# apache/arrow-go

Hardware: AMD Instinct MI355X
Metric: GB/s processed per kernel (Sum/Add/Filter/Take) vs HBM roofline (higher is better)
Workload: dtype int64+f64

## Files before the change

### arrow_go_amd/csrc/ah_common.h

```cpp
#pragma once
#include <hip/hip_runtime.h>
#include <initializer_list>
#include <type_traits>
#include <stdarg.h>
#include <stdint.h>
#include <stddef.h>
#include <stdio.h>
#include <stdlib.h>
#include <string.h>
#include "../../include/arrowhip.h"

#define AH_EXPORT extern "C" __attribute__((visibility("default")))

struct ah_filter_cache {
  bool valid;
  const uint8_t *fdata, *fvalid;
  int64_t foff, n, ntiles;
  int null_sel, tile_rows;
  void* buf;
  size_t bytes;
  int64_t* super_off;
  int* tile_local;
  int64_t* total;
};
// ... 71 lines not shown
static inline int ah_fail(ah_ctx* ctx, int code, const char* fmt, ...) {
  if (ctx) {
    va_list ap;
    va_start(ap, fmt);
    vsnprintf(ctx->err, sizeof(ctx->err), fmt, ap);
    va_end(ap);
  }
  return code;
}

#define AH_HIP(ctx, call)                                                              \
  do {                                                                                 \
    hipError_t e__ = (call);                                                           \
    if (e__ != hipSuccess)                                                             \
      return ah_fail((ctx), AH_EHIP, "%s failed: %s (%s:%d)", #call, hipGetErrorString(e__), \
                     __FILE__, __LINE__);                                              \
  } while (0)

#define AH_ENTER_KEEP(ctx)                                             \
  do {                                                                 \
    if (!(ctx)) return AH_EINVALID;                                    \
    (ctx)->err[0] = 0;                                                 \
    AH_HIP((ctx), hipSetDevice((ctx)->device));                        \
  } while (0)

#define AH_ENTER(ctx)                                                  \
  do {                                                                 \
    AH_ENTER_KEEP(ctx);                                                \
    (ctx)->fcache.valid = false;                                       \
    (ctx)->take_hint_valid = false;                                    \
  } while (0)

static inline bool ah_take_hint_overlaps(const ah_ctx* c, const void* p, size_t nbytes) {
  if (!c->take_hint_valid || !c->take_hint_idx) return false;
  const uintptr_t a = (uintptr_t)p, b = a + nbytes, lo = (uintptr_t)c->take_hint_idx, hi = lo + (size_t)c->take_hint_nidx * (size_t)(c->take_hint_kind / 2);
  return a < hi && lo < b;
}
static inline bool ah_fcache_overlaps(const ah_ctx* c, const void* p, size_t nbytes) {
  if (!c->fcache.valid) return false;
  const uintptr_t a = (uintptr_t)p, b = a + nbytes;
  const uintptr_t lo = (uintptr_t)(c->fcache.foff >> 3), hi = (uintptr_t)((c->fcache.foff + c->fcache.n + 7) >> 3);
  for (const uint8_t* bm : {c->fcache.fdata, c->fcache.fvalid})
    if (bm && a < (uintptr_t)bm + hi && (uintptr_t)bm + lo < b) return true;
  return false;
}

#define AH_LAUNCH_CHECK(ctx) AH_HIP((ctx), hipGetLastError())

void ah_expr_cache_free(ah_ctx* ctx);
int ah_arith_binary(ah_ctx* ctx, int type, int op, int shape, const void* l, const void* r, void* out, int64_t len);
int ah_partition_by_group(ah_ctx* ctx, const int32_t* ids, const unsigned long long* vals, const uint8_t* vvalid, int64_t voff, int64_t n,
                          int shift, int passes, unsigned* hist, unsigned* offs, unsigned long long* alt_vals, unsigned* alt_ids,
                          unsigned long long* out_vals, unsigned* out_ids);
int ah_sort_rest_msd(ah_ctx* ctx, unsigned long long* keys, unsigned* rows, unsigned long long* alt_keys, unsigned* alt_rows, int64_t n,
                     unsigned long long varying, unsigned long long kmin, unsigned long long kmax, int float_bytes, int descending, void* tmp,
                     unsigned long long* out64, int* used);
size_t ah_sort_msd_temp_bytes(int64_t n);
int ah_sort_pairs_lsd(ah_ctx* ctx, unsigned long long* keys, unsigned* rows, unsigned long long* alt_keys, unsigned* alt_rows, int64_t n,
                      unsigned* hist, unsigned* offs, unsigned long long** sorted_keys);
int ah_take_binned_try(ah_ctx* ctx, int byte_width, const void* values, const uint8_t* vvalid, int64_t voff, int64_t nvalues, int iw,
                       int is_signed, const void* idx, const uint8_t* ivalid, int64_t ioff, int64_t nidx, void* out_values,
                       uint8_t* out_valid, unsigned long long* first_bad, int* used);
int ah_groupby_partitioned_try(ah_ctx* ctx, int is_f64, const uint64_t* keys, const uint8_t* kvalid, int64_t koff, const void* vals,
                               const uint8_t* vvalid, int64_t voff, int64_t n, uint64_t* out_keys, void* out_sums, int64_t* out_counts,
                               int64_t* out_first_rows, int64_t* out_ngroups, int32_t* out_null_group, int* used);
int ah_fused_f64_parts_dev(ah_ctx* ctx, int cmpop, const double* x, const uint8_t* valid, int64_t off, int64_t n, double threshold,
                           double* out_sum_dev, int64_t* out_count_dev, double* out_parts_dev);
size_t ah_sum_partial_bytes(int is_f64);
int ah_sum_chunk_partials(ah_ctx* ctx, int is_f64, const void* buf, size_t len, void* partials, int max_partials, int* n_written);
int ah_sum_finish_partials(ah_ctx* ctx, int is_f64, const void* partials, int n, void* res_dev);
int ah_sum_short_f64(ah_ctx* ctx, const void* buf, size_t len, void* res_dev);
int ah_encode_partitioned_try(ah_ctx* ctx, const uint64_t* keys, const uint8_t* valid, int64_t off, int64_t n, int encode_nulls, int lp, int slots,
                              int32_t* out_ids, uint64_t* out_dict, int64_t* out_first_rows, int64_t* out_ndict, int32_t* out_null_id, int* used);
int ah_encode_u64_groups(ah_ctx* ctx, const uint64_t* keys, const uint8_t* kvalid, int64_t koff, int64_t n, int32_t* ids, uint64_t* out_keys,
                         int64_t* out_first_rows, int64_t* out_ngroups, int32_t* out_null_group);
int ah_encode_u64_first_seen(ah_ctx* ctx, const uint64_t* keys, const uint8_t* valid, int64_t off, int64_t n, int32_t* ids, int64_t* out_first_rows,
                             int64_t* out_ngroups);
int ah_encode_tuple_first_seen(ah_ctx* ctx, int ncols, const ah_group_key* keys, int64_t n, int32_t* ids, int64_t* out_first_rows, int64_t* out_ngroups);
int ah_encode_first_look(ah_ctx* ctx, const uint64_t* keys, const uint8_t* valid, int64_t off, int64_t rows, uint64_t* distinct);
int ah_encode_partitioned2_try(ah_ctx* ctx, const uint64_t* keys, const uint8_t* valid, int64_t off, int64_t n, int encode_nulls, int lp, int slots,
                               int32_t* out_ids, uint64_t* out_dict, int64_t* out_first_rows, int64_t* out_ndict, int32_t* out_null_id, int* used);
int ah_compact_u64_by_bits(ah_ctx* ctx, const uint64_t* values, const uint8_t* bits, int64_t n, uint64_t* out_values, int64_t* out_rows);
int ah_check_stall(ah_ctx* ctx);
int ah_mailbox_read(ah_ctx* ctx, const unsigned long long* dev_words, int nwords, unsigned long long* out_host);
int ah_mailbox_begin(ah_ctx* ctx, unsigned long long** mb_out, unsigned long long* seq_out);
int ah_mailbox_wait(ah_ctx* ctx, unsigned long long seq, int nwords, unsigned long long* out_host);
#if defined(__HIPCC__)
__device__ __forceinline__ void ah_mailbox_post(unsigned long long* mb, unsigned long long seq, const unsigned long long* words, int nwords) {
  for (int i = 0; i < nwords; i++) __hip_atomic_store(&mb[i], words[i], __ATOMIC_RELAXED, __HIP_MEMORY_SCOPE_SYSTEM);
  __hip_atomic_store(&mb[7], seq, __ATOMIC_RELEASE, __HIP_MEMORY_SCOPE_SYSTEM);
}
#endif
int ah_mailbox_read2(ah_ctx* ctx, const unsigned long long* dev_words, int nwords, const unsigned long long* dev_words2, int nwords2,
                     unsigned long long* out_host);
int ah_scratch_reserve(ah_ctx* ctx, size_t nbytes, void** out);
int ah_temp_reserve(ah_ctx* ctx, size_t nbytes, void** out, bool* out_of_memory = nullptr);
int ah_pack_reserve(ah_ctx* ctx, size_t nbytes, void** out);
static inline constexpr size_t ah_pad(size_t b) { return (b + 255) & ~(size_t)255; }
struct TempCarver {
  uint8_t* base = nullptr;
  size_t used = 0;
  uint8_t* take(size_t b) { uint8_t* q = base ? base + used : nullptr; used += ah_pad(b); return q; }
  template <typename T> size_t take(T*& p, size_t count) { p = (T*)take(count * sizeof(T)); return ah_pad(count * sizeof(T)); }
};
constexpr int kDsScalars = 64;
constexpr int kDsSum = 0;
constexpr int kDsFusedSum = 8, kDsFusedCount = 9;
constexpr int kDsMinMax = 12;
constexpr int kDsGbDone = 20;
// ... 210 lines not shown
```

### arrow_go_amd/csrc/ah_sort.hip

```cpp
#include <algorithm>
#include <type_traits>
#include <vector>
#include "ah_sort_radix.h"

namespace {

enum { kCatRest = 0, kCatNaN = 1, kCatNull = 2 };

template <typename T>
__device__ __forceinline__ unsigned long long make_key(T v, bool descending) {
  using U = typename std::make_unsigned<typename std::conditional<std::is_floating_point<T>::value,
                                                                    typename std::conditional<sizeof(T) == 4, int, long long>::type, T>::type>::type;
  constexpr U sign = (U)1 << (sizeof(T) * 8 - 1);
  U k;
  if constexpr (std::is_floating_point<T>::value) {
    if (v == (T)0) v = (T)0;
    U b = __builtin_bit_cast(U, v);
    k = (b & sign) ? (U)~b : (U)(b | sign);
  } else if constexpr (std::is_signed<T>::value) {
    k = (U)v ^ sign;
  } else {
    k = (U)v;
  }
  if (descending) k = (U)~k;
  return (unsigned long long)k;
}

template <typename T>
struct Column {
  const T* values;
  const uint8_t* valid;
  int64_t off;
  int descending, nulls_at_start;
  const unsigned* rows_in;
  __device__ __forceinline__ void load(int64_t i, unsigned long long* key, unsigned* row, unsigned* digit) const {
    const unsigned r = rows_in ? rows_in[i] : (unsigned)i;
    const T v = values[r];
    int cat = kCatRest;
    if (!ah_bit(valid, off + r)) cat = kCatNull;
    else if (std::is_floating_point<T>::value && v != v) cat = kCatNaN;
    *key = cat == kCatRest ? make_key<T>(v, descending) : 0ull;
    *row = r;
    *digit = nulls_at_start ? (unsigned)(2 - cat) : (unsigned)cat;
  }
};
struct IdVal {
  const int32_t* ids;
  const unsigned long long* vals;
  const uint8_t* vvalid;
  int64_t voff;
  int shift;
  __device__ __forceinline__ void load(int64_t i, unsigned long long* key, unsigned* row, unsigned* digit) const {
    const unsigned g = (unsigned)ids[i];
    const bool ok = ah_bit(vvalid, voff + i);
    *key = ok ? vals[i] : 0ull;
    *row = ok ? g : (g | 0x80000000u);
    *digit = (g >> shift) & 255u;
  }
};

struct ValId {
  const unsigned long long* vals;
  const unsigned* ids;
  int shift;
  __device__ __forceinline__ void load(int64_t i, unsigned long long* key, unsigned* row, unsigned* digit) const {
    *key = vals[i];
    *row = ids[i];
    *digit = ((*row & 0x7fffffffu) >> shift) & 255u;
  }
};

template <typename T>
__global__ __launch_bounds__(kBlock) void pairs_kernel(const T* __restrict__ values, int64_t n, int descending, unsigned long long* __restrict__ keys,
                                                        unsigned* __restrict__ rows, unsigned long long* __restrict__ res) {
  KeyStats st;
  st.init();
  constexpr int U = 4;
  const int64_t stride = (int64_t)gridDim.x * kBlock * U;
  for (int64_t base = (int64_t)blockIdx.x * kBlock * U + threadIdx.x; base < n; base += stride) {
    T v[U];
#pragma unroll
    for (int u = 0; u < U; u++) { const int64_t i = base + (int64_t)u * kBlock; v[u] = i < n ? __builtin_nontemporal_load(&values[i]) : (T)0; }
#pragma unroll
    for (int u = 0; u < U; u++) {
      const int64_t i = base + (int64_t)u * kBlock;
      if (i >= n) continue;
      if (std::is_floating_point<T>::value && v[u] != v[u]) { st.nans++; continue; }
      const unsigned long long k = make_key<T>(v[u], descending);
      __builtin_nontemporal_store(k, &keys[i]);
      __builtin_nontemporal_store((unsigned)i, &rows[i]);
      st.add(k);
    }
  }
  st = ah_block_reduce<kBlock>(st);
  if (threadIdx.x == 0) st.store<5>(res + (size_t)blockIdx.x * 5);
}

__global__ __launch_bounds__(kBlock) void emit_kernel(const unsigned* __restrict__ rows, int64_t n, uint64_t* __restrict__ out) {
  const int64_t stride = (int64_t)gridDim.x * kBlock;
  for (int64_t i = (int64_t)blockIdx.x * kBlock + threadIdx.x; i < n; i += stride) out[i] = rows[i];
}


template <typename T>
int sort_by_column(ah_ctx* c, SortBuffers& b, const void* values, const uint8_t* valid, int64_t off, int64_t n, int descending,
                   int nulls_at_start, const unsigned* rows_in) {
  const int64_t ntiles = ah_ceil_div(n, (int64_t)kTile * tiles_per_block(n));
  int rc;
  Column<T> col{(const T*)values, valid, off, descending, nulls_at_start, rows_in};
  int64_t rest_lo = 0, rest_n = 0;
  unsigned long long k_and = ~0ull, k_or = 0, kmin = ~0ull, kmax = 0;
  bool have_stats = false;
  if (valid == nullptr && rows_in == nullptr && n >= ((int64_t)1 << 20)) {
    const unsigned pgrid = std::min(ah_stream_grid(c, ah_ceil_div(n, (int64_t)kBlock * 4), 8), (unsigned)kAndOrGrid);
    pairs_kernel<T><<<pgrid, kBlock, 0, c->stream>>>((const T*)values, n, descending, b.ka, b.ra, b.andor);
    AH_LAUNCH_CHECK(c);
    std::vector<unsigned long long> parts((size_t)pgrid * 5);
    AH_HIP(c, hipMemcpyAsync(parts.data(), b.andor, parts.size() * 8, hipMemcpyDeviceToHost, c->stream));
    AH_HIP(c, hipStreamSynchronize(c->stream));
    unsigned long long nans = 0;
    for (unsigned g = 0; g < pgrid; g++) {
      k_and &= parts[g * 5]; k_or |= parts[g * 5 + 1];
      kmin = parts[g * 5 + 2] < kmin ? parts[g * 5 + 2] : kmin;
      kmax = parts[g * 5 + 3] > kmax ? parts[g * 5 + 3] : kmax;
      nans += parts[g * 5 + 4];
    }
    if (nans == 0) { have_stats = true; rest_lo = 0; rest_n = n; }
  }
  if (!have_stats) {
    if ((rc = radix_pass(c, col, n, b.hist, b.offs, b.ka, b.ra)) != AH_OK) return rc;
    unsigned ends[3];
    for (int d = 0; d < 3; d++)
      AH_HIP(c, hipMemcpyAsync(&c->pinned[d], b.offs + ((int64_t)d + 1) * ntiles - 1, 4, hipMemcpyDeviceToHost, c->stream));
    AH_HIP(c, hipStreamSynchronize(c->stream));
    for (int d = 0; d < 3; d++) ends[d] = *(volatile unsigned*)&c->pinned[d];
    rest_lo = nulls_at_start ? ends[1] : 0;
    rest_n = nulls_at_start ? (int64_t)ends[2] - ends[1] : ends[0];
  }
  unsigned long long *kcur = b.ka + rest_lo, *kalt = b.kb + rest_lo;
  unsigned *rcur = b.ra + rest_lo, *ralt = b.rb + rest_lo;
  if (rest_n > 1) {
    if (!have_stats) {
      const unsigned agrid = std::min(ah_stream_grid(c, ah_ceil_div(rest_n, kBlock), 4), (unsigned)kAndOrGrid);
      and_or_kernel<<<agrid, kBlock, 0, c->stream>>>(kcur, rest_n, b.andor);
      AH_LAUNCH_CHECK(c);
      std::vector<unsigned long long> parts((size_t)agrid * 4);
      AH_HIP(c, hipMemcpyAsync(parts.data(), b.andor, parts.size() * 8, hipMemcpyDeviceToHost, c->stream));
      AH_HIP(c, hipStreamSynchronize(c->stream));
      for (unsigned g = 0; g < agrid; g++) {
        k_and &= parts[g * 4]; k_or |= parts[g * 4 + 1];
        kmin = parts[g * 4 + 2] < kmin ? parts[g * 4 + 2] : kmin;
        kmax = parts[g * 4 + 3] > kmax ? parts[g * 4 + 3] : kmax;
      }
    }
    const unsigned long long varying = k_and ^ k_or;
    int nvar = 0;
    for (int by = 0; by < (int)sizeof(T); by++) nvar += ((varying >> (8 * by)) & 0xFFull) != 0;
    bool done = false;
    if (rows_in == nullptr && nvar >= 4 && c->opt_sort_msd) {
      int used = -1;
      if ((rc = ah_sort_rest_msd(c, kcur, rcur, kalt, ralt, rest_n, varying, kmin, kmax, std::is_floating_point<T>::value ? (int)sizeof(T) : 0, descending, b.msd_tmp,
                                 (unsigned long long*)(rest_n == n ? b.final_out : nullptr), &used)) != AH_OK) return rc;
      if (used > 0) {
        done = true;
        b.emitted = rest_n == n && b.final_out != nullptr;
      } else if (used == 0 && b.msd_tmp && ah_sort_msd_temp_bytes(rest_n) != 0) {
        if ((rc = radix_pass(c, col, n, b.hist, b.offs, b.ka, b.ra)) != AH_OK) return rc;
      }
    }
    for (int by = 0; !done && by < (int)sizeof(T); by++) {
      if (((varying >> (8 * by)) & 0xFFull) == 0) continue;
      Pairs src{kcur, rcur, 8 * by};
      if ((rc = radix_pass(c, src, rest_n, b.hist, b.offs, kalt, ralt)) != AH_OK) return rc;
      unsigned long long* tk = kcur; kcur = kalt; kalt = tk;
      unsigned* tr = rcur; rcur = ralt; ralt = tr;
    }
    if (!b.emitted && rcur != b.ra + rest_lo) AH_HIP(c, hipMemcpyAsync(b.ra + rest_lo, rcur, (size_t)rest_n * 4, hipMemcpyDeviceToDevice, c->stream));
  }
  return AH_OK;
}

int sort_dispatch(ah_ctx* c, SortBuffers& b, const SortCol& k, int64_t n, const unsigned* rows_in) {
  switch (k.type) {
#define AH_SORT(ID, T) case ID: return sort_by_column<T>(c, b, k.values, k.valid, k.off, n, k.descending, k.nulls_at_start, rows_in);
    AH_SORT(AH_UINT8, uint8_t) AH_SORT(AH_INT8, int8_t) AH_SORT(AH_UINT16, uint16_t) AH_SORT(AH_INT16, int16_t)
    AH_SORT(AH_UINT32, uint32_t) AH_SORT(AH_INT32, int32_t) AH_SORT(AH_UINT64, uint64_t) AH_SORT(AH_INT64, int64_t)
    AH_SORT(AH_FLOAT32, float) AH_SORT(AH_FLOAT64, double)
#undef AH_SORT
  }
  if (ah_sort_is_binary(k.type)) return ah_sort_by_binary(c, b, k, n, rows_in);
  return ah_fail(c, AH_ENOTIMPL, "sorting not supported for type %d", k.type);
}

int sort_keys(ah_ctx* c, int nkeys, const SortCol* keys, int64_t n, uint64_t* out) {
  SortBuffers b;
  const int64_t ntiles = ah_ceil_div(n, kTile);
  int rc;
  bool any_binary = false;
  for (int k = 0; k < nkeys; k++) any_binary |= ah_sort_is_binary(keys[k].type);
  const size_t hist_bytes = (size_t)kRadix * ntiles * 4;
  const size_t msd_bytes = c->opt_sort_msd ? ah_sort_msd_temp_bytes(n) : 0;
  const size_t bin_bytes = any_binary ? kBinArrays * Carver::pad((size_t)n * 4) : 0;
  const size_t total = 2 * Carver::pad((size_t)n * 8) + (nkeys > 1 ? 3 : 2) * Carver::pad((size_t)n * 4) + 2 * Carver::pad(hist_bytes) + Carver::pad(4096 * 8 * 8) + Carver::pad(msd_bytes) + bin_bytes;
  void* arena;
  if ((rc = ah_temp_reserve(c, total, &arena)) != AH_OK) return rc;
  Carver tmp{(uint8_t*)arena};
  tmp.take((size_t)n * 8, &b.ka);
  tmp.take((size_t)n * 8, &b.kb);
  tmp.take((size_t)n * 4, &b.ra);
  tmp.take((size_t)n * 4, &b.rb);
  b.rc = nullptr;
  if (nkeys > 1) tmp.take((size_t)n * 4, &b.rc);
  tmp.take(hist_bytes, &b.hist);
  tmp.take(hist_bytes, &b.offs);
  tmp.take((size_t)kAndOrGrid * 8 * 8, &b.andor);
  if (msd_bytes) { uint8_t* m; tmp.take(msd_bytes, &m); b.msd_tmp = m; }
  if (any_binary)
    for (int i = 0; i < kBinArrays; i++) tmp.take((size_t)n * 4, &b.bin[i]);
  const unsigned* rows_in = nullptr;
  if (nkeys == 1) b.final_out = out;
  for (int k = nkeys - 1; k >= 0; k--) {
    if ((rc = sort_dispatch(c, b, keys[k], n, rows_in)) != AH_OK) return rc;
    if (k > 0) {
      AH_HIP(c, hipMemcpyAsync(b.rc, b.ra, (size_t)n * 4, hipMemcpyDeviceToDevice, c->stream));
      rows_in = b.rc;
    }
  }
  if (!b.emitted) {
    emit_kernel<<<ah_stream_grid(c, ah_ceil_div(n, kBlock), 8), kBlock, 0, c->stream>>>(b.ra, n, out);
    AH_LAUNCH_CHECK(c);
  }
  return AH_OK;
}

}

int ah_partition_by_group(ah_ctx* c, const int32_t* ids, const unsigned long long* vals, const uint8_t* vvalid, int64_t voff, int64_t n, int shift,
// ... 99 lines not shown
```

### arrow_go_amd/csrc/ah_sort_msd.hip

```cpp
#include "ah_common.h"
#include "ah_bins.h"
#include "ah_msd.h"

namespace {

constexpr int kLocalMax = 512;
constexpr int kBigMax = 8192, kBigList = 1024;

struct MsMap {
  unsigned long long mask;
  int lshift;
  int fkind, descending;
};
__device__ __forceinline__ double ms_value(unsigned long long u, const MsMap& m) {
  if (m.fkind == 8) {
    const unsigned long long k = m.descending ? ~u : u;
    return __builtin_bit_cast(double, (k >> 63) ? (k & 0x7fffffffffffffffull) : ~k);
  }
  const unsigned k = m.descending ? ~(unsigned)(u >> 32) : (unsigned)(u >> 32);
  return (double)__builtin_bit_cast(float, (k >> 31) ? (k & 0x7fffffffu) : ~k);
}
__device__ __forceinline__ double ms_frac(unsigned long long u, unsigned long long pa, unsigned long long pb, const MsMap& m) {
  if (pb <= pa) return 0.0;
  if (m.fkind && m.lshift == (m.fkind == 8 ? 0 : 32) && ((pa ^ pb) >> 63)) {
    const double xa = ms_value(pa, m), xb = ms_value(pb, m);
    if (xb != xa && xa - xa == 0.0 && xb - xb == 0.0) return (ms_value(u, m) - xa) / (xb - xa);
  }
  return (double)(u - pa) / (double)(pb - pa);
}
constexpr int kSplit = 4096;
constexpr int64_t kSample = (int64_t)1 << 18;

__global__ __launch_bounds__(256) void ms_sample_kernel(const unsigned long long* __restrict__ keys, int64_t n, int64_t stride, int64_t count, MsMap m,
                                                         unsigned long long* __restrict__ sample, unsigned* __restrict__ sample_rows) {
  const int64_t j = (int64_t)blockIdx.x * 256 + threadIdx.x;
  if (j >= count) return;
  const int64_t i = j * stride;
  sample[j] = i < n ? (keys[i] & m.mask) << m.lshift : ~0ull;
  sample_rows[j] = (unsigned)j;
}
struct MsPoints {
  const unsigned long long* sorted;
  int64_t count;
  unsigned long long umin, umax;
  __device__ __forceinline__ unsigned long long at(int64_t i) const { return i <= 0 ? umin : (i > count ? umax : sorted[i - 1]); }
  __device__ __forceinline__ int64_t first(int k) const { return k == 0 ? 0 : 64 * (int64_t)k + 1; }
  __device__ __forceinline__ int64_t last(int k) const { return k == kSplit - 1 ? count + 1 : 64 * (int64_t)(k + 1) + 1; }
};
constexpr int kFlagWords = kSplit / 32;
__global__ __launch_bounds__(256) void ms_split_kernel(MsPoints p, unsigned long long* __restrict__ split, unsigned* __restrict__ flags) {
  const int k = blockIdx.x * 256 + threadIdx.x;
  if (k > kSplit) return;
  split[k] = k == kSplit ? p.umax : p.at(p.first(k));
  if (k == kSplit) return;
  const int64_t i0 = p.first(k), i1 = p.last(k);
  const unsigned long long a = p.at(i0), b = p.at(i1);
  bool flag = k == 0 || k == kSplit - 1;
  if (!flag && b > a) {
    const double w = (double)(b - a), g = (double)(i1 - i0);
    for (int64_t i = i0 + 1; i < i1; i++) {
      const double dev = (double)(p.at(i) - a) / w - (double)(i - i0) / g;
      flag = flag || dev > 0.25 || dev < -0.25;
    }
  }
  if (flag) atomicOr(&flags[k >> 5], 1u << (k & 31));
}

__global__ __launch_bounds__(256) void ms_dupes_kernel(const unsigned long long* __restrict__ sorted, int64_t count, int64_t run, unsigned* __restrict__ found) {
  const int64_t i = (int64_t)blockIdx.x * 256 + threadIdx.x;
  if (i + run < count && sorted[i] == sorted[i + run]) *found = 1u;
}

__global__ __launch_bounds__(256) void ms_guide_kernel(const unsigned long long* __restrict__ split, unsigned short* __restrict__ guide) {
  const int c = blockIdx.x * 256 + threadIdx.x;
  if (c > 4096) return;
  if (c == 4096) { guide[c] = (unsigned short)(kSplit - 1); return; }
  const unsigned long long v = (unsigned long long)c << 52;
  int lo = 0;
  for (int step = kSplit >> 1; step > 0; step >>= 1) lo += split[lo + step] <= v ? step : 0;
  guide[c] = (unsigned short)lo;
}

__global__ __launch_bounds__(kThreads) void ms_bucket_kernel(const unsigned long long* __restrict__ keys, int64_t n, MsMap m, MsPoints p,
                                                         const unsigned long long* __restrict__ split, const unsigned* __restrict__ flags,
                                                         const unsigned short* __restrict__ guide, unsigned per, unsigned* __restrict__ bucket) {
  __shared__ unsigned long long s_s[kSplit + 1];
  __shared__ unsigned s_f[kFlagWords];
  __shared__ unsigned short s_g[4097];
  for (int i = threadIdx.x; i <= kSplit; i += kThreads) { s_s[i] = split[i]; s_g[i] = guide[i]; }
  for (int i = threadIdx.x; i < kFlagWords; i += kThreads) s_f[i] = flags[i];
  __syncthreads();
  constexpr int U = 4;
  const int64_t stride = (int64_t)gridDim.x * kThreads * U;
  for (int64_t base = (int64_t)blockIdx.x * kThreads * U + threadIdx.x; base < n; base += stride) {
    unsigned long long u[U];
    unsigned lo[U], hi[U];
#pragma unroll
    for (int q = 0; q < U; q++) {
      const int64_t i = base + q * kThreads;
      u[q] = i < n ? (__builtin_nontemporal_load(&keys[i]) & m.mask) << m.lshift : s_s[0];
    }
#pragma unroll
    for (int q = 0; q < U; q++) { lo[q] = s_g[u[q] >> 52]; hi[q] = s_g[(u[q] >> 52) + 1]; }
    bool more = true;
    while (more) {
      more = false;
#pragma unroll
      for (int q = 0; q < U; q++) {
        if (lo[q] < hi[q]) {
          const unsigned mid = (lo[q] + hi[q] + 1) >> 1;
          if (s_s[mid] <= u[q]) lo[q] = mid; else hi[q] = mid - 1;
          more = more || lo[q] < hi[q];
        }
      }
    }
#pragma unroll
    for (int q = 0; q < U; q++) {
      const int64_t i = base + q * kThreads;
      if (i >= n) continue;
      double f;
      if ((s_f[lo[q] >> 5] >> (lo[q] & 31)) & 1u) {
        int64_t a = p.first((int)lo[q]), b = p.last((int)lo[q]);
        const double g = (double)(b - a);
        const int64_t a0 = a;
        unsigned long long pa = p.at(a), pb = p.at(b);
        while (b - a > 1) {
          const int64_t mid = (a + b) >> 1;
          const unsigned long long pm = p.at(mid);
          if (b - a <= 16) {
            const double d = ms_frac(pm, pa, pb, m) - (double)(mid - a) / (double)(b - a);
            if (d < 0.3 && d > -0.3) break;
          }
          if (pm <= u[q]) { a = mid; pa = pm; } else { b = mid; pb = pm; }
        }
        f = ((double)(a - a0) + ms_frac(u[q], pa, pb, m) * (double)(b - a)) / g;
      } else {
        const unsigned long long x = s_s[lo[q]], y = s_s[lo[q] + 1];
        f = y > x ? (double)(u[q] - x) * __builtin_amdgcn_rcp((double)(y - x)) : 0.0;
      }
      f = f >= 0.0 ? f : 0.0;
      unsigned in = (unsigned)(f * (double)per);
      in = in < per ? in : per - 1;
      __builtin_nontemporal_store(lo[q] * per + in, &bucket[i]);
    }
  }
}

struct MsDigit {
  static constexpr int kMaxDigits = kMaxNb2;
  const unsigned* bucket; int shift; unsigned mask;
  __device__ __forceinline__ unsigned digit(int64_t i, int) const { return (__builtin_nontemporal_load(&bucket[i]) >> shift) & mask; }
};

template <bool WITH_BUCKET>
__global__ __launch_bounds__(kThreads) void ms_scatter_kernel(const unsigned long long* __restrict__ keys, const unsigned* __restrict__ rows,
                                                               const unsigned* __restrict__ bucket, int64_t n, const unsigned* __restrict__ pstart,
                                                               int nparents, int shift, unsigned mask, int nb, const unsigned* __restrict__ toffs,
                                                               unsigned long long* __restrict__ out_keys, unsigned* __restrict__ out_rows,
                                                               unsigned* __restrict__ out_bucket) {
  __shared__ unsigned s_cnt[kMaxNb2], s_start[kMaxNb2], s_goff[kMaxNb2], s_wsum[kThreads / 64];
  __shared__ unsigned s_a[kThreads], s_b[kThreads];
  __shared__ unsigned long long s_stage[kMsTile];
  __shared__ uint16_t s_bin[kMsTile];
  __shared__ int s_pick;
  __shared__ unsigned s_carry;
  const TileRange r = ms_tile(pstart, nparents, n, s_a, s_b, s_wsum, &s_pick);
  if (r.parent < 0) return;
  const int t = threadIdx.x;
  for (int b = t; b < nb; b += kThreads) s_cnt[b] = 0;
  unsigned long long k[kMsRows];
  unsigned rw[kMsRows], bk[kMsRows], dg[kMsRows], rank[kMsRows];
  bool live[kMsRows];
#pragma unroll
  for (int u = 0; u < kMsRows; u++) {
    const int64_t i = r.lo + u * kThreads + t;
    live[u] = i < r.hi;
    k[u] = live[u] ? __builtin_nontemporal_load(&keys[i]) : 0ull;
    rw[u] = live[u] ? __builtin_nontemporal_load(&rows[i]) : 0u;
    bk[u] = live[u] ? __builtin_nontemporal_load(&bucket[i]) : 0u;
  }
  __syncthreads();
#pragma unroll
  for (int u = 0; u < kMsRows; u++) {
    dg[u] = (bk[u] >> shift) & mask;
    rank[u] = live[u] ? atomicAdd(&s_cnt[dg[u]], 1u) : 0u;
  }
  __syncthreads();
  digit_excl_scan(s_cnt, nb, s_a, s_b, s_wsum, &s_carry, [&](int d, unsigned st) {
    s_start[d] = st;
    s_goff[d] = toffs[r.id * nb + d] - st;
  });
  const int tile_n = (int)(r.hi - r.lo);
#pragma unroll
  for (int u = 0; u < kMsRows; u++)
    if (live[u]) { const unsigned q = s_start[dg[u]] + rank[u]; s_stage[q] = k[u]; s_bin[q] = (uint16_t)dg[u]; }
  __syncthreads();
  int64_t dst[kMsRows];
#pragma unroll
  for (int u = 0; u < kMsRows; u++) {
    const int q = u * kThreads + t;
    dst[u] = q < tile_n ? (int64_t)s_goff[s_bin[q]] + q : -1;
    if (dst[u] >= 0) out_keys[dst[u]] = s_stage[q];
  }
  __syncthreads();
  unsigned* s_stage32 = reinterpret_cast<unsigned*>(s_stage);
#pragma unroll
  for (int u = 0; u < kMsRows; u++)
    if (live[u]) { const unsigned q = s_start[dg[u]] + rank[u]; s_stage32[q] = rw[u]; if (WITH_BUCKET) s_stage32[kMsTile + q] = bk[u]; }
  __syncthreads();
#pragma unroll
  for (int u = 0; u < kMsRows; u++)
    if (dst[u] >= 0) {
      out_rows[dst[u]] = s_stage32[u * kThreads + t];
      if (WITH_BUCKET) out_bucket[dst[u]] = s_stage32[kMsTile + u * kThreads + t];
    }
}

struct KR {
  unsigned long long k;
  unsigned r;
  static __device__ __forceinline__ bool less(const KR& a, const KR& b) { return a.k < b.k || (a.k == b.k && a.r < b.r); }
  static __device__ __forceinline__ KR xchg(const KR& a, int j, int lane) {
    KR o;
    o.k = ((unsigned long long)ms_xor_lane((unsigned)(a.k >> 32), j, lane) << 32) | ms_xor_lane((unsigned)a.k, j, lane);
    o.r = ms_xor_lane(a.r, j, lane);
    return o;
  }
};
__device__ __forceinline__ bool kr_less(const KR& a, const KR& b) { return KR::less(a, b); }
struct C64 {
  unsigned long long c;
// ... 96 lines not shown
  else ms_sort_bucket<8>(keys, rows, s, m, lane, out_rows, out64);
}

__global__ __launch_bounds__(kThreads) void ms_big_kernel(const unsigned long long* __restrict__ keys, const unsigned* rows,
                                                           const unsigned* __restrict__ bstart, const unsigned* __restrict__ oversize,
                                                           const unsigned* __restrict__ big_list, unsigned* out_rows,
                                                           unsigned long long* __restrict__ out64) {
  __shared__ unsigned long long s_k[kBigMax];
  __shared__ unsigned s_r[kBigMax];
  if (blockIdx.x >= oversize[1] || blockIdx.x >= (unsigned)kBigList) return;
  const unsigned b = big_list[blockIdx.x], s = bstart[b];
  const int m = (int)(bstart[b + 1] - s);
  int p2 = 1024;
  while (p2 < m) p2 <<= 1;
  for (int i = threadIdx.x; i < p2; i += kThreads) { s_k[i] = i < m ? keys[s + i] : ~0ull; s_r[i] = i < m ? rows[s + i] : ~0u; }
  __syncthreads();
  for (int k = 2; k <= p2; k <<= 1) {
    for (int j = k >> 1; j > 0; j >>= 1) {
      for (int i = threadIdx.x; i < p2; i += kThreads) {
        const int q = i ^ j;
        if (q > i) {
          const KR x{s_k[i], s_r[i]}, y{s_k[q], s_r[q]};
          const bool asc = (i & k) == 0;
          if (kr_less(y, x) == asc) { s_k[i] = y.k; s_r[i] = y.r; s_k[q] = x.k; s_r[q] = x.r; }
        }
      }
      __syncthreads();
    }
  }
  for (int i = threadIdx.x; i < m; i += kThreads) { if (out64) out64[s + i] = s_r[i]; else out_rows[s + i] = s_r[i]; }
}

}

static void ms_plan(int64_t n, int* lb_out, int* lb2_out) {
  int lb = 0;
  while (((int64_t)64 << lb) < n) lb++;
  if (lb > 21) lb = 21;
  *lb_out = lb;
  *lb2_out = lb >= 20 ? lb - 10 : lb - lb / 2;
}

size_t ah_sort_msd_temp_bytes(int64_t n) {
  if (n < ((int64_t)1 << 22) || n > ((int64_t)1 << 27)) return 0;
  int lb, lb2;
  ms_plan(n, &lb, &lb2);
  const int nb2 = 1 << lb2, nb1 = 1 << (lb - lb2);
  const int64_t ntiles = ah_ceil_div(n, kMsTile), ngrp = ah_ceil_div(ntiles, kGroupTiles), nvt = ((ntiles + nb1 + 7) / 8) * 8;
  return ah_pad((size_t)n * 4) * 2 + ah_pad((size_t)kSample * 8) * 2 + ah_pad((size_t)kSample * 4) * 2 + ah_pad((size_t)(kSplit + 1) * 8) + ah_pad(kFlagWords * 4) + ah_pad(4097 * 2) +
         ah_pad((size_t)ntiles * nb1 * 4) * 2 + ah_pad((size_t)ngrp * nb1 * 4) + ah_pad((size_t)(nb1 + 1) * 4) + ah_pad((size_t)nvt * nb2 * 4) * 2 +
         ah_pad(((size_t)1 << lb) * 4 + 4) + ah_pad((size_t)kBigList * 4) + 256;
}

int ah_sort_rest_msd(ah_ctx* c, unsigned long long* keys, unsigned* rows, unsigned long long* alt_keys, unsigned* alt_rows, int64_t n,
                     unsigned long long varying, unsigned long long kmin, unsigned long long kmax, int float_bytes, int descending, void* tmp,
                     unsigned long long* out64, int* used) {
  *used = -1;
  if (!tmp || varying == 0 || ah_sort_msd_temp_bytes(n) == 0) return AH_OK;
  unsigned* out_rows = rows;
  int lb, lb2;
  ms_plan(n, &lb, &lb2);
  const int nb2 = 1 << lb2, nb1 = 1 << (lb - lb2);
  const unsigned nbuckets = 1u << lb;
  const int hb = 63 - __builtin_clzll(varying);
  MsMap map{hb == 63 ? ~0ull : ((1ull << (hb + 1)) - 1), 63 - hb, float_bytes, descending};
  const int64_t ntiles = ah_ceil_div(n, kMsTile), ngrp = ah_ceil_div(ntiles, kGroupTiles), nvt = ((ntiles + nb1 + 7) / 8) * 8;
  const unsigned grid1 = (unsigned)(((ntiles + 7) / 8) * 8);
  const int64_t sample_n = n < kSample ? n : kSample;
  TempCarver tc;
  tc.base = (uint8_t*)tmp;
  int rc;
  unsigned* bucket = (unsigned*)tc.take((size_t)n * 4);
  unsigned* bucket2 = (unsigned*)tc.take((size_t)n * 4);
  unsigned long long* sample = (unsigned long long*)tc.take((size_t)kSample * 8);
  unsigned long long* sample_alt = (unsigned long long*)tc.take((size_t)kSample * 8);
  unsigned* sample_rows = (unsigned*)tc.take((size_t)kSample * 4);
  unsigned* sample_rows_alt = (unsigned*)tc.take((size_t)kSample * 4);
  unsigned long long* split = (unsigned long long*)tc.take((size_t)(kSplit + 1) * 8);
  unsigned* flags = (unsigned*)tc.take(kFlagWords * 4);
  unsigned short* guide = (unsigned short*)tc.take(4097 * 2);
  unsigned* cnt1 = (unsigned*)tc.take((size_t)ntiles * nb1 * 4);
  unsigned* toffs1 = (unsigned*)tc.take((size_t)ntiles * nb1 * 4);
  unsigned* gsum = (unsigned*)tc.take((size_t)ngrp * nb1 * 4);
  unsigned* pstart = (unsigned*)tc.take((size_t)(nb1 + 1) * 4);
  unsigned* cnt2 = (unsigned*)tc.take((size_t)nvt * nb2 * 4);
  unsigned* toffs2 = (unsigned*)tc.take((size_t)nvt * nb2 * 4);
  unsigned* bstart = (unsigned*)tc.take(((size_t)nbuckets + 1) * 4);
  unsigned* big_list = (unsigned*)tc.take((size_t)kBigList * 4);
  unsigned* oversize = (unsigned*)&c->dscalars[26];
  AH_HIP(c, hipMemsetAsync(oversize, 0, 8, c->stream));
  ms_sample_kernel<<<(unsigned)ah_ceil_div(sample_n, 256), 256, 0, c->stream>>>(keys, n, n / sample_n, sample_n, map, sample, sample_rows);
  AH_LAUNCH_CHECK(c);
  unsigned long long* sorted = nullptr;
  if ((rc = ah_sort_pairs_lsd(c, sample, sample_rows, sample_alt, sample_rows_alt, sample_n, (unsigned*)cnt2, (unsigned*)toffs2, &sorted)) != AH_OK) return rc;
  {
    const int64_t run = (int64_t)(kBigMax / 2) * sample_n / n;
    ms_dupes_kernel<<<(unsigned)ah_ceil_div(sample_n, 256), 256, 0, c->stream>>>(sorted, sample_n, run < 1 ? 1 : run, oversize);
    AH_LAUNCH_CHECK(c);
    AH_HIP(c, hipMemcpyAsync(&c->pinned[12], oversize, 8, hipMemcpyDeviceToHost, c->stream));
    AH_HIP(c, hipStreamSynchronize(c->stream));
    if (((volatile unsigned*)&c->pinned[12])[0] != 0) {
      if (getenv("ARROWHIP_DEBUG_MSD")) fprintf(stderr, "msd: n=%lld: the sample shows a key with more than %d rows, not attempted\n", (long long)n, kBigMax / 2);
      *used = -1;
      return AH_OK;
    }
  }
  *used = 0;
  MsPoints pts{sorted, sample_n, (kmin & map.mask) << map.lshift, (kmax & map.mask) << map.lshift};
  AH_HIP(c, hipMemsetAsync(flags, 0, kFlagWords * 4, c->stream));
  ms_split_kernel<<<(kSplit + 256) / 256, 256, 0, c->stream>>>(pts, split, flags);
  AH_LAUNCH_CHECK(c);
  ms_guide_kernel<<<17, 256, 0, c->stream>>>(split, guide);
  AH_LAUNCH_CHECK(c);
  ms_bucket_kernel<<<ah_stream_grid(c, ah_ceil_div(n, kThreads * 4), 2), kThreads, 0, c->stream>>>(keys, n, map, pts, split, flags, guide, nbuckets / kSplit, bucket);
  AH_LAUNCH_CHECK(c);
  tile_hist_kernel<MsDigit><<<grid1, kThreads, 0, c->stream>>>(MsDigit{bucket, lb2, (unsigned)(nb1 - 1)}, n, nullptr, 1, nb1, cnt1);
  AH_LAUNCH_CHECK(c);
  if ((rc = launch_tile_offsets(c, cnt1, nb1, ntiles, n, gsum, toffs1, pstart)) != AH_OK) return rc;
  ms_scatter_kernel<true><<<grid1, kThreads, 0, c->stream>>>(keys, rows, bucket, n, nullptr, 1, lb2, (unsigned)(nb1 - 1), nb1, toffs1, alt_keys,
                                                                        alt_rows, bucket2);
  AH_LAUNCH_CHECK(c);
  tile_hist_kernel<MsDigit><<<(unsigned)nvt, kThreads, 0, c->stream>>>(MsDigit{bucket2, 0, (unsigned)(nb2 - 1)}, n, pstart, nb1, nb2, cnt2);
  AH_LAUNCH_CHECK(c);
  ms_offs2_kernel<<<(unsigned)nb1, kThreads, 0, c->stream>>>(cnt2, pstart, nb1, nb2, toffs2, bstart, n);
  AH_LAUNCH_CHECK(c);
  ms_scatter_kernel<false><<<(unsigned)nvt, kThreads, 0, c->stream>>>(alt_keys, alt_rows, bucket2, n, pstart, nb1, 0, (unsigned)(nb2 - 1), nb2, toffs2, keys,
                                                                      rows, nullptr);
  AH_LAUNCH_CHECK(c);
  ms_local_kernel<<<(unsigned)ah_ceil_div((int64_t)nbuckets, 4), 256, 0, c->stream>>>(keys, rows, bstart, (int64_t)nbuckets, out_rows, out64, oversize, big_list);
  AH_LAUNCH_CHECK(c);
  ms_big_kernel<<<kBigList, kThreads, 0, c->stream>>>(keys, rows, bstart, oversize, big_list, out_rows, out64);
  AH_LAUNCH_CHECK(c);
  AH_HIP(c, hipMemcpyAsync(&c->pinned[12], oversize, 8, hipMemcpyDeviceToHost, c->stream));
  AH_HIP(c, hipStreamSynchronize(c->stream));
  const unsigned too_big = ((volatile unsigned*)&c->pinned[12])[0], listed = ((volatile unsigned*)&c->pinned[12])[1];
  if (getenv("ARROWHIP_DEBUG_MSD")) fprintf(stderr, "msd: n=%lld lb=%d nb1=%d nb2=%d largest unsortable bucket=%u, buckets sorted by a workgroup=%u\n", (long long)n, lb, nb1, nb2, too_big, listed);
  if (too_big != 0 || listed > (unsigned)kBigList) return AH_OK;
  *used = 1;
  return AH_OK;
}
```

Before: 6302.

## Read sort keys straight from the column in MSD path instead of materializing pairs

When the MSD sort path will be taken, the stats kernel no longer writes the key and row arrays. The MSD sample, bucket and first scatter kernels now compute keys on the fly from the source column, and row ids come from the index. This avoids one full write and read of the key/row pair buffers. If MSD declines, the pair arrays are generated afterwards, which adds an extra pass over the column on that fallback path.

Result: no change. 6394 (median of 2 runs) (+1.5%).

```diff
diff --git a/arrow_go_amd/csrc/ah_common.h b/arrow_go_amd/csrc/ah_common.h
--- a/arrow_go_amd/csrc/ah_common.h
+++ b/arrow_go_amd/csrc/ah_common.h
@@ -147,9 +147,9 @@
 int ah_partition_by_group(ah_ctx* ctx, const int32_t* ids, const unsigned long long* vals, const uint8_t* vvalid, int64_t voff, int64_t n,
                           int shift, int passes, unsigned* hist, unsigned* offs, unsigned long long* alt_vals, unsigned* alt_ids,
                           unsigned long long* out_vals, unsigned* out_ids);
-int ah_sort_rest_msd(ah_ctx* ctx, unsigned long long* keys, unsigned* rows, unsigned long long* alt_keys, unsigned* alt_rows, int64_t n,
-                     unsigned long long varying, unsigned long long kmin, unsigned long long kmax, int float_bytes, int descending, void* tmp,
-                     unsigned long long* out64, int* used);
+int ah_sort_rest_msd(ah_ctx* ctx, unsigned long long* keys, unsigned* rows, const void* column, int column_type, unsigned long long* alt_keys,
+                     unsigned* alt_rows, int64_t n, unsigned long long varying, unsigned long long kmin, unsigned long long kmax, int float_bytes,
+                     int descending, void* tmp, unsigned long long* out64, int* used);
 size_t ah_sort_msd_temp_bytes(int64_t n);
 int ah_sort_pairs_lsd(ah_ctx* ctx, unsigned long long* keys, unsigned* rows, unsigned long long* alt_keys, unsigned* alt_rows, int64_t n,
                       unsigned* hist, unsigned* offs, unsigned long long** sorted_keys);
diff --git a/arrow_go_amd/csrc/ah_sort.hip b/arrow_go_amd/csrc/ah_sort.hip
--- a/arrow_go_amd/csrc/ah_sort.hip
+++ b/arrow_go_amd/csrc/ah_sort.hip
@@ -2,29 +2,11 @@
 #include <type_traits>
 #include <vector>
 #include "ah_sort_radix.h"
+#include "ah_sort_key.h"
 
 namespace {
 
 enum { kCatRest = 0, kCatNaN = 1, kCatNull = 2 };
-
-template <typename T>
-__device__ __forceinline__ unsigned long long make_key(T v, bool descending) {
-  using U = typename std::make_unsigned<typename std::conditional<std::is_floating_point<T>::value,
-                                                                    typename std::conditional<sizeof(T) == 4, int, long long>::type, T>::type>::type;
-  constexpr U sign = (U)1 << (sizeof(T) * 8 - 1);
-  U k;
-  if constexpr (std::is_floating_point<T>::value) {
-    if (v == (T)0) v = (T)0;
-    U b = __builtin_bit_cast(U, v);
-    k = (b & sign) ? (U)~b : (U)(b | sign);
-  } else if constexpr (std::is_signed<T>::value) {
-    k = (U)v ^ sign;
-  } else {
-    k = (U)v;
-  }
-  if (descending) k = (U)~k;
-  return (unsigned long long)k;
-}
 
 template <typename T>
 struct Column {
@@ -87,8 +69,10 @@
       if (i >= n) continue;
       if (std::is_floating_point<T>::value && v[u] != v[u]) { st.nans++; continue; }
       const unsigned long long k = make_key<T>(v[u], descending);
-      __builtin_nontemporal_store(k, &keys[i]);
-      __builtin_nontemporal_store((unsigned)i, &rows[i]);
+      if (keys) {
+        __builtin_nontemporal_store(k, &keys[i]);
+        __builtin_nontemporal_store((unsigned)i, &rows[i]);
+      }
       st.add(k);
     }
   }
@@ -103,7 +87,7 @@
 
 
 template <typename T>
-int sort_by_column(ah_ctx* c, SortBuffers& b, const void* values, const uint8_t* valid, int64_t off, int64_t n, int descending,
+int sort_by_column(ah_ctx* c, SortBuffers& b, int type, const void* values, const uint8_t* valid, int64_t off, int64_t n, int descending,
                    int nulls_at_start, const unsigned* rows_in) {
   const int64_t ntiles = ah_ceil_div(n, (int64_t)kTile * tiles_per_block(n));
   int rc;
@@ -111,9 +95,12 @@
   int64_t rest_lo = 0, rest_n = 0;
   unsigned long long k_and = ~0ull, k_or = 0, kmin = ~0ull, kmax = 0;
   bool have_stats = false;
+  bool pairs_stored = true;
+  unsigned pgrid = 0;
   if (valid == nullptr && rows_in == nullptr && n >= ((int64_t)1 << 20)) {
-    const unsigned pgrid = std::min(ah_stream_grid(c, ah_ceil_div(n, (int64_t)kBlock * 4), 8), (unsigned)kAndOrGrid);
-    pairs_kernel<T><<<pgrid, kBlock, 0, c->stream>>>((const T*)values, n, descending, b.ka, b.ra, b.andor);
+    pgrid = std::min(ah_stream_grid(c, ah_ceil_div(n, (int64_t)kBlock * 4), 8), (unsigned)kAndOrGrid);
+    pairs_stored = !(sizeof(T) >= 4 && c->opt_sort_msd && ah_sort_msd_temp_bytes(n) != 0);
+    pairs_kernel<T><<<pgrid, kBlock, 0, c->stream>>>((const T*)values, n, descending, pairs_stored ? b.ka : nullptr, b.ra, b.andor);
     AH_LAUNCH_CHECK(c);
     std::vector<unsigned long long> parts((size_t)pgrid * 5);
     AH_HIP(c, hipMemcpyAsync(parts.data(), b.andor, parts.size() * 8, hipMemcpyDeviceToHost, c->stream));
@@ -129,6 +116,7 @@
   }
   if (!have_stats) {
     if ((rc = radix_pass(c, col, n, b.hist, b.offs, b.ka, b.ra)) != AH_OK) return rc;
+    pairs_stored = true;
     unsigned ends[3];
     for (int d = 0; d < 3; d++)
       AH_HIP(c, hipMemcpyAsync(&c->pinned[d], b.offs + ((int64_t)d + 1) * ntiles - 1, 4, hipMemcpyDeviceToHost, c->stream));
@@ -159,14 +147,20 @@
     bool done = false;
     if (rows_in == nullptr && nvar >= 4 && c->opt_sort_msd) {
       int used = -1;
-      if ((rc = ah_sort_rest_msd(c, kcur, rcur, kalt, ralt, rest_n, varying, kmin, kmax, std::is_floating_point<T>::value ? (int)sizeof(T) : 0, descending, b.msd_tmp,
+      if ((rc = ah_sort_rest_msd(c, kcur, rcur, pairs_stored ? nullptr : values, type, kalt, ralt, rest_n, varying, kmin, kmax, std::is_floating_point<T>::value ? (int)sizeof(T) : 0, descending, b.msd_tmp,
                                  (unsigned long long*)(rest_n == n ? b.final_out : nullptr), &used)) != AH_OK) return rc;
       if (used > 0) {
         done = true;
         b.emitted = rest_n == n && b.final_out != nullptr;
       } else if (used == 0 && b.msd_tmp && ah_sort_msd_temp_bytes(rest_n) != 0) {
         if ((rc = radix_pass(c, col, n, b.hist, b.offs, b.ka, b.ra)) != AH_OK) return rc;
+        pairs_stored = true;
       }
+    }
+    if (!done && !pairs_stored) {
+      pairs_kernel<T><<<pgrid, kBlock, 0, c->stream>>>((const T*)values, n, descending, b.ka, b.ra, b.andor);
+      AH_LAUNCH_CHECK(c);
+      pairs_stored = true;
     }
     for (int by = 0; !done && by < (int)sizeof(T); by++) {
       if (((varying >> (8 * by)) & 0xFFull) == 0) continue;
@@ -182,7 +176,7 @@
 
 int sort_dispatch(ah_ctx* c, SortBuffers& b, const SortCol& k, int64_t n, const unsigned* rows_in) {
   switch (k.type) {
-#define AH_SORT(ID, T) case ID: return sort_by_column<T>(c, b, k.values, k.valid, k.off, n, k.descending, k.nulls_at_start, rows_in);
+#define AH_SORT(ID, T) case ID: return sort_by_column<T>(c, b, ID, k.values, k.valid, k.off, n, k.descending, k.nulls_at_start, rows_in);
     AH_SORT(AH_UINT8, uint8_t) AH_SORT(AH_INT8, int8_t) AH_SORT(AH_UINT16, uint16_t) AH_SORT(AH_INT16, int16_t)
     AH_SORT(AH_UINT32, uint32_t) AH_SORT(AH_INT32, int32_t) AH_SORT(AH_UINT64, uint64_t) AH_SORT(AH_INT64, int64_t)
     AH_SORT(AH_FLOAT32, float) AH_SORT(AH_FLOAT64, double)
diff --git a/arrow_go_amd/csrc/ah_sort_key.h b/arrow_go_amd/csrc/ah_sort_key.h
--- /dev/null
+++ b/arrow_go_amd/csrc/ah_sort_key.h
@@ -0,0 +1,26 @@
+#pragma once
+#include <type_traits>
+#include "ah_common.h"
+
+namespace {
+
+template <typename T>
+__device__ __forceinline__ unsigned long long make_key(T v, bool descending) {
+  using U = typename std::make_unsigned<typename std::conditional<std::is_floating_point<T>::value,
+                                                                    typename std::conditional<sizeof(T) == 4, int, long long>::type, T>::type>::type;
+  constexpr U sign = (U)1 << (sizeof(T) * 8 - 1);
+  U k;
+  if constexpr (std::is_floating_point<T>::value) {
+    if (v == (T)0) v = (T)0;
+    U b = __builtin_bit_cast(U, v);
+    k = (b & sign) ? (U)~b : (U)(b | sign);
+  } else if constexpr (std::is_signed<T>::value) {
+    k = (U)v ^ sign;
+  } else {
+    k = (U)v;
+  }
+  if (descending) k = (U)~k;
+  return (unsigned long long)k;
+}
+
+}
diff --git a/arrow_go_amd/csrc/ah_sort_msd.hip b/arrow_go_amd/csrc/ah_sort_msd.hip
--- a/arrow_go_amd/csrc/ah_sort_msd.hip
+++ b/arrow_go_amd/csrc/ah_sort_msd.hip
@@ -1,8 +1,20 @@
 #include "ah_common.h"
 #include "ah_bins.h"
 #include "ah_msd.h"
+#include "ah_sort_key.h"
 
 namespace {
+
+struct StoredKeys {
+  const unsigned long long* keys;
+  __device__ __forceinline__ unsigned long long key(int64_t i) const { return __builtin_nontemporal_load(&keys[i]); }
+};
+template <typename T>
+struct ColumnKeys {
+  const T* values;
+  int descending;
+  __device__ __forceinline__ unsigned long long key(int64_t i) const { return make_key<T>(__builtin_nontemporal_load(&values[i]), descending); }
+};
 
 constexpr int kLocalMax = 512;
 constexpr int kBigMax = 8192, kBigList = 1024;
@@ -31,12 +43,13 @@
 constexpr int kSplit = 4096;
 constexpr int64_t kSample = (int64_t)1 << 18;
 
-__global__ __launch_bounds__(256) void ms_sample_kernel(const unsigned long long* __restrict__ keys, int64_t n, int64_t stride, int64_t count, MsMap m,
+template <typename SRC>
+__global__ __launch_bounds__(256) void ms_sample_kernel(SRC src, int64_t n, int64_t stride, int64_t count, MsMap m,
                                                          unsigned long long* __restrict__ sample, unsigned* __restrict__ sample_rows) {
   const int64_t j = (int64_t)blockIdx.x * 256 + threadIdx.x;
   if (j >= count) return;
   const int64_t i = j * stride;
-  sample[j] = i < n ? (keys[i] & m.mask) << m.lshift : ~0ull;
+  sample[j] = i < n ? (src.key(i) & m.mask) << m.lshift : ~0ull;
   sample_rows[j] = (unsigned)j;
 }
 struct MsPoints {
@@ -81,7 +94,8 @@
   guide[c] = (unsigned short)lo;
 }
 
-__global__ __launch_bounds__(kThreads) void ms_bucket_kernel(const unsigned long long* __restrict__ keys, int64_t n, MsMap m, MsPoints p,
+template <typename SRC>
+__global__ __launch_bounds__(kThreads) void ms_bucket_kernel(SRC src, int64_t n, MsMap m, MsPoints p,
                                                          const unsigned long long* __restrict__ split, const unsigned* __restrict__ flags,
                                                          const unsigned short* __restrict__ guide, unsigned per, unsigned* __restrict__ bucket) {
   __shared__ unsigned long long s_s[kSplit + 1];
@@ -98,7 +112,7 @@
 #pragma unroll
     for (int q = 0; q < U; q++) {
       const int64_t i = base + q * kThreads;
-      u[q] = i < n ? (__builtin_nontemporal_load(&keys[i]) & m.mask) << m.lshift : s_s[0];
+      u[q] = i < n ? (src.key(i) & m.mask) << m.lshift : s_s[0];
     }
 #pragma unroll
     for (int q = 0; q < U; q++) { lo[q] = s_g[u[q] >> 52]; hi[q] = s_g[(u[q] >> 52) + 1]; }
@@ -152,8 +166,8 @@
   __device__ __forceinline__ unsigned digit(int64_t i, int) const { return (__builtin_nontemporal_load(&bucket[i]) >> shift) & mask; }
 };
 
-template <bool WITH_BUCKET>
-__global__ __launch_bounds__(kThreads) void ms_scatter_kernel(const unsigned long long* __restrict__ keys, const unsigned* __restrict__ rows,
+template <bool WITH_BUCKET, typename SRC>
+__global__ __launch_bounds__(kThreads) void ms_scatter_kernel(SRC src, const unsigned* __restrict__ rows,
                                                                const unsigned* __restrict__ bucket, int64_t n, const unsigned* __restrict__ pstart,
                                                                int nparents, int shift, unsigned mask, int nb, const unsigned* __restrict__ toffs,
                                                                unsigned long long* __restrict__ out_keys, unsigned* __restrict__ out_rows,
@@ -175,8 +189,8 @@
   for (int u = 0; u < kMsRows; u++) {
     const int64_t i = r.lo + u * kThreads + t;
     live[u] = i < r.hi;
-    k[u] = live[u] ? __builtin_nontemporal_load(&keys[i]) : 0ull;
-    rw[u] = live[u] ? __builtin_nontemporal_load(&rows[i]) : 0u;
+    k[u] = live[u] ? src.key(i) : 0ull;
+    rw[u] = !live[u] ? 0u : rows ? __builtin_nontemporal_load(&rows[i]) : (unsigned)i;
     bk[u] = live[u] ? __builtin_nontemporal_load(&bucket[i]) : 0u;
   }
   __syncthreads();
@@ -379,9 +393,11 @@
          ah_pad(((size_t)1 << lb) * 4 + 4) + ah_pad((size_t)kBigList * 4) + 256;
 }
 
-int ah_sort_rest_msd(ah_ctx* c, unsigned long long* keys, unsigned* rows, unsigned long long* alt_keys, unsigned* alt_rows, int64_t n,
-                     unsigned long long varying, unsigned long long kmin, unsigned long long kmax, int float_bytes, int descending, void* tmp,
-                     unsigned long long* out64, int* used) {
+namespace {
+template <typename SRC>
+int rest_msd(ah_ctx* c, SRC src, bool rows_stored, unsigned long long* keys, unsigned* rows, unsigned long long* alt_keys, unsigned* alt_rows,
+             int64_t n, unsigned long long varying, unsigned long long kmin, unsigned long long kmax, int float_bytes, int descending,
+             void* tmp, unsigned long long* out64, int* used) {
   *used = -1;
   if (!tmp || varying == 0 || ah_sort_msd_temp_bytes(n) == 0) return AH_OK;
   unsigned* out_rows = rows;
@@ -416,7 +432,7 @@
   unsigned* big_list = (unsigned*)tc.take((size_t)kBigList * 4);
   unsigned* oversize = (unsigned*)&c->dscalars[26];
   AH_HIP(c, hipMemsetAsync(oversize, 0, 8, c->stream));
-  ms_sample_kernel<<<(unsigned)ah_ceil_div(sample_n, 256), 256, 0, c->stream>>>(keys, n, n / sample_n, sample_n, map, sample, sample_rows);
+  ms_sample_kernel<SRC><<<(unsigned)ah_ceil_div(sample_n, 256), 256, 0, c->stream>>>(src, n, n / sample_n, sample_n, map, sample, sample_rows);
   AH_LAUNCH_CHECK(c);
   unsigned long long* sorted = nullptr;
   if ((rc = ah_sort_pairs_lsd(c, sample, sample_rows, sample_alt, sample_rows_alt, sample_n, (unsigned*)cnt2, (unsigned*)toffs2, &sorted)) != AH_OK) return rc;
@@ -439,19 +455,19 @@
   AH_LAUNCH_CHECK(c);
   ms_guide_kernel<<<17, 256, 0, c->stream>>>(split, guide);
   AH_LAUNCH_CHECK(c);
-  ms_bucket_kernel<<<ah_stream_grid(c, ah_ceil_div(n, kThreads * 4), 2), kThreads, 0, c->stream>>>(keys, n, map, pts, split, flags, guide, nbuckets / kSplit, bucket);
+  ms_bucket_kernel<SRC><<<ah_stream_grid(c, ah_ceil_div(n, kThreads * 4), 2), kThreads, 0, c->stream>>>(src, n, map, pts, split, flags, guide, nbuckets / kSplit, bucket);
   AH_LAUNCH_CHECK(c);
   tile_hist_kernel<MsDigit><<<grid1, kThreads, 0, c->stream>>>(MsDigit{bucket, lb2, (unsigned)(nb1 - 1)}, n, nullptr, 1, nb1, cnt1);
   AH_LAUNCH_CHECK(c);
   if ((rc = launch_tile_offsets(c, cnt1, nb1, ntiles, n, gsum, toffs1, pstart)) != AH_OK) return rc;
-  ms_scatter_kernel<true><<<grid1, kThreads, 0, c->stream>>>(keys, rows, bucket, n, nullptr, 1, lb2, (unsigned)(nb1 - 1), nb1, toffs1, alt_keys,
-                                                                        alt_rows, bucket2);
+  ms_scatter_kernel<true, SRC><<<grid1, kThreads, 0, c->stream>>>(src, rows_stored ? rows : nullptr, bucket, n, nullptr, 1, lb2, (unsigned)(nb1 - 1), nb1,
+                                                                             toffs1, alt_keys, alt_rows, bucket2);
   AH_LAUNCH_CHECK(c);
   tile_hist_kernel<MsDigit><<<(unsigned)nvt, kThreads, 0, c->stream>>>(MsDigit{bucket2, 0, (unsigned)(nb2 - 1)}, n, pstart, nb1, nb2, cnt2);
   AH_LAUNCH_CHECK(c);
   ms_offs2_kernel<<<(unsigned)nb1, kThreads, 0, c->stream>>>(cnt2, pstart, nb1, nb2, toffs2, bstart, n);
   AH_LAUNCH_CHECK(c);
-  ms_scatter_kernel<false><<<(unsigned)nvt, kThreads, 0, c->stream>>>(alt_keys, alt_rows, bucket2, n, pstart, nb1, 0, (unsigned)(nb2 - 1), nb2, toffs2, keys,
+  ms_scatter_kernel<false, StoredKeys><<<(unsigned)nvt, kThreads, 0, c->stream>>>(StoredKeys{alt_keys}, alt_rows, bucket2, n, pstart, nb1, 0, (unsigned)(nb2 - 1), nb2, toffs2, keys,
                                                                       rows, nullptr);
   AH_LAUNCH_CHECK(c);
   ms_local_kernel<<<(unsigned)ah_ceil_div((int64_t)nbuckets, 4), 256, 0, c->stream>>>(keys, rows, bstart, (int64_t)nbuckets, out_rows, out64, oversize, big_list);
@@ -466,3 +482,18 @@
   *used = 1;
   return AH_OK;
 }
+}
+
+int ah_sort_rest_msd(ah_ctx* c, unsigned long long* keys, unsigned* rows, const void* column, int column_type, unsigned long long* alt_keys,
+                     unsigned* alt_rows, int64_t n, unsigned long long varying, unsigned long long kmin, unsigned long long kmax, int float_bytes,
+                     int descending, void* tmp, unsigned long long* out64, int* used) {
+  if (!column) return rest_msd(c, StoredKeys{keys}, true, keys, rows, alt_keys, alt_rows, n, varying, kmin, kmax, float_bytes, descending, tmp, out64, used);
+  switch (column_type) {
+#define AH_MSD_COLUMN(ID, T) \
+  case ID: return rest_msd(c, ColumnKeys<T>{(const T*)column, descending}, false, keys, rows, alt_keys, alt_rows, n, varying, kmin, kmax, float_bytes, descending, tmp, out64, used);
+    AH_MSD_COLUMN(AH_UINT32, uint32_t) AH_MSD_COLUMN(AH_INT32, int32_t) AH_MSD_COLUMN(AH_UINT64, uint64_t) AH_MSD_COLUMN(AH_INT64, int64_t)
+    AH_MSD_COLUMN(AH_FLOAT32, float) AH_MSD_COLUMN(AH_FLOAT64, double)
+#undef AH_MSD_COLUMN
+  }
+  return ah_fail(c, AH_EINVALID, "sort_indices: no MSD path over a column of type %d", column_type);
+}
```
